# devmentality/LEAStereo

Hardware: AMD Instinct MI355X
Metric: stereo pairs/s at 576×960 D=192, 1/2/4/8 GPU; EPE vs reference (higher is better)
Workload: dtype f32; 1 GPU; SceneFlow 576x960 D=192 fp32, batch 1 per GPU (BASELINE configs[1]); height=576, width=960, maxdisp=192, global_batch=1, parallelism=dp1 (pairs sharded over ranks, no collective in the step), launch=hip graph replay

## Files before the change

### include/leastereo_hip.h

```cpp
#ifndef LEASTEREO_HIP_H
#define LEASTEREO_HIP_H

#include <stddef.h>
#include <stdint.h>

#ifdef __cplusplus
extern "C" {
#endif

#define LEA_ABI_VERSION 14

#define LEA_F32 0
#define LEA_BF16 1

#define LEA_OK 0
#define LEA_E_INVALID 1001
#define LEA_E_UNSUPPORTED 1002

#define LEA_RELU 1u
#define LEA_RESIDUAL 2u
#define LEA_PAIR_SUM 4u

int lea_abi_version(void);
const char* lea_last_error(void);
// ... 15 lines not shown
                      unsigned flags, int dtype, void* stream);

int lea_conv3d_bnrelu_resampled(const void* x, int64_t x_bstride, int Di, int Hi, int Wi,
                                const float* w_packed, const float* scale, const float* shift,
                                const void* residual, int64_t r_bstride,
                                void* y, int64_t y_bstride,
                                int B, int cin, int cout, int D, int H, int W, int k,
                                unsigned flags, int dtype, void* stream);

int lea_conv3d_bnrelu_costvolume(const void* left, const void* right, int64_t f_bstride,
                                 const float* w_packed, const float* scale, const float* shift,
                                 void* y, int64_t y_bstride, int B, int C, int cout, int D3,
                                 int H, int W, unsigned flags, int dtype, void* stream);
const char* lea_conv3d_costvolume_kernel_name(int B, int cout, int D3, int H, int W);

const char* lea_conv3d_kernel_name(int B, int cout, int D, int H, int W, int k, int resampled);


size_t lea_conv2d_packed_floats(int cout, int cin);
int lea_conv2d_pack_weights(const float* w, float* packed, int cout, int cin, void* stream);

int lea_conv2d_bnrelu(const void* x, int64_t x_bstride, const float* w_packed,
                      const float* scale, const float* shift, const void* residual,
                      int64_t r_bstride, void* y, int64_t y_bstride, int B, int cin, int cout,
                      int H, int W, unsigned flags, int dtype, void* stream);

const char* lea_conv2d_kernel_name(int B, int cout, int H, int W);

int lea_conv2d_bnrelu_pair(const void* x, int64_t x_bstride, const float* w_packed,
                           const float* scale, const float* shift, const void* residual,
                           int64_t r_bstride, void* y, int64_t y_bstride, void* y2,
                           int64_t y2_bstride, int B, int cin, int cout, int c1, int H, int W,
                           unsigned flags, void* stream);

int lea_conv2d_s3_bnrelu(const void* x, int64_t x_bstride, const float* w, const float* scale,
                         const float* shift, void* y, int64_t y_bstride, int B, int cin, int cout,
                         int Hi, int Wi, unsigned flags, int dtype, void* stream);

int lea_feature_stem_bnrelu(const float* x, int64_t x_bstride, const float* w0, const float* scale0,
                            const float* shift0, const float* w1, const float* scale1,
                            const float* shift1, void* y, int64_t y_bstride, int B, int cin, int c0,
                            int c1, int Hi, int Wi, int dtype, void* stream);


int lea_resample3d_trilinear(const void* x, int64_t x_bstride, void* y, int64_t y_bstride,
                             int B, int C, int Di, int Hi, int Wi, int Do, int Ho, int Wo,
                             int align_corners, const float* scale, const float* shift,
                             unsigned flags, int dtype, void* stream);

size_t lea_tapsum_workspace_bytes(int B, int cout, int Hi, int Wi, int Do);
int lea_tapsum_upsample(const void* q, int64_t q_bstride, void* y, int64_t y_bstride,
                        int B, int cout, int Di, int Hi, int Wi, int Do, int Ho, int Wo,
                        const float* scale, const float* shift, unsigned flags,
                        void* workspace, int dtype, void* stream);

int lea_disparity_regression(const void* cost, float* disp, int B, int D3, int H3, int W3,
                             int maxdisp, int dtype, void* stream);

int lea_disparity_regression_stats(const void* cost, float* disp, float* entropy, float* peak,
                                   float* disp_local, int B, int D3, int H3, int W3, int maxdisp,
                                   int radius, int dtype, void* stream);

int lea_disparity_regression_right(const void* cost, float* disp_right, int B, int D3, int H3,
                                   int W3, int maxdisp, int dtype, void* stream);

int lea_disparity_lr_check(const float* disp_left, const float* disp_right, uint8_t* state,
// ... 220 lines not shown
```

### include/leastereo_hip_tuning.h

```cpp
#ifndef LEASTEREO_HIP_TUNING_H
#define LEASTEREO_HIP_TUNING_H

#ifdef __cplusplus
extern "C" {
#endif

int lea_conv3d_set_tile_override(int nt, int tw, int td);

int lea_conv3d_set_rs_gather(int on);

int lea_conv1x1_set_vector(int on);

int lea_conv3d_bf16_set_tile_override(int th, int td, int mt);

int lea_conv3d_bf16_set_variant(int variant);

int lea_conv3d_bf16_set_stream1x1(int on);

int lea_conv3d_bf16_set_pair_split(int on);

int lea_resample_bf16_set_batch(int k);

int lea_resample_bf16_set_cols(int on);

int lea_resample_set_mode(int mode);

int lea_conv2d_set_small(int on);

const char* lea_conv2d_kernel_name_cin(int B, int cin, int cout, int H, int W);

int lea_disparity_set_register_form(int on);

int lea_tapsum_set_rows(int on);

int lea_staged_rows(int Hi, int Ho, int ac, int R, int halo);

int lea_conv3d_wino_set_w22(int on);

int lea_conv3d_wino_set_tile_override(int np, int td, int f);

int lea_conv3d_wino_set_variant(int variant);

int lea_conv3d_wino2_set_walk(int spw);

int lea_conv3d_wino2_set_halo16(int on);

int lea_conv3d_wino2_set_lane_halo16(int on);

int lea_conv3d_wino_set_fence(int on);

int lea_conv3d_wino2_set_pipeline(int on);

int lea_conv3d_wino2p_set_wpre(int on);

int lea_conv3d_wino44_set(int on);

int lea_conv3d_wino44_set_upre(int on);

int lea_conv3d_wino44_set_sched(int s);

int lea_conv3d_wino44_set_group(int g);

// ... 11 lines not shown
```

### leastereo_amd/_lib.py

```python
from __future__ import annotations

import ctypes
import os
import threading

LIB_PATH = os.environ.get(
    "LEASTEREO_HIP_LIB",
    os.path.join(os.path.dirname(os.path.abspath(__file__)), "libleastereo_hip.so"))

ABI_VERSION = 14
LEA_F32 = 0
LEA_BF16 = 1
LEA_RELU = 1
LEA_RESIDUAL = 2
LEA_PAIR_SUM = 4
LEA_E_INVALID = 1001

_p = ctypes.c_void_p
_i = ctypes.c_int
_i64 = ctypes.c_int64
_u = ctypes.c_uint

SIGNATURES = {
    "lea_abi_version": (_i, []),
# ... 75 lines not shown
    "lea_from_c8_bf16": (_i, [_p, _i64, _p, _i64, _i, _i, _i64, _p]),
    "lea_conv3d_wino_packed_floats": (ctypes.c_size_t, [_i, _i]),
    "lea_conv3d_wino_pack_weights": (_i, [_p, _p, _i, _i, _p]),
    "lea_conv3d_bnrelu_wino": (_i, [_p, _i64, _p, _i64, _i, _p, _p, _p, _p, _i64, _p, _i64,
                                    _i, _i, _i, _i, _i, _i, _u, _i, _p]),
    "lea_conv3d_bnrelu_costvolume_wino": (_i, [_p, _p, _i64, _p, _p, _p, _p, _i64, _i, _i, _i,
                                               _i, _i, _i, _u, _i, _p]),
    "lea_conv3d_wino_kernel_name": (ctypes.c_char_p, [_i, _i, _i, _i, _i, _i, _i]),
    "lea_conv3d_wino_down2_supported": (_i, [_i, _i, _i, _i, _i, _i]),
    "lea_conv3d_wino_down2_kernel_name": (ctypes.c_char_p, [_i, _i, _i, _i, _i, _i]),
    "lea_conv3d_bnrelu_wino_down2": (_i, [_p, _i64, _p, _p, _p, _p, _i64, _i, _i, _i, _i, _i, _i, _u, _i, _p]),
    "lea_conv3d_wino_down2_cat_supported": (_i, [_i, _i, _i, _i, _i, _i, _i]),
    "lea_conv3d_wino_down2_cat_kernel_name": (ctypes.c_char_p, [_i, _i, _i, _i, _i, _i, _i]),
    "lea_conv3d_bnrelu_wino_down2_cat": (_i, [_p, _i64, _p, _i64, _i, _p, _p, _p, _p, _i64, _i, _i, _i, _i, _i, _i,
                                              _u, _i, _p]),
    "lea_conv3d_wino_dp_down2_supported": (_i, [_i, _i, _i, _i, _i, _i]),
    "lea_conv3d_wino_dp_down2_kernel_name": (ctypes.c_char_p, [_i, _i, _i, _i, _i, _i, _i]),
    "lea_conv3d_bnrelu_wino_dp_down2": (_i, [_p, _i64, _p, _p, _p, _p, _i64, _p, _i64, _p, _i64, _i, _i, _i, _i, _i,
                                             _i, _u, _i, _p]),
    "lea_resample3d_down2_supported": (_i, [_i, _i, _i, _i, _i, _i, _i]),
    "lea_resample3d_trilinear_down2": (_i, [_p, _i64, _p, _i64, _p, _i64, _i, _i, _i, _i, _i, _i, _i, _i, _p, _p,
                                            _u, _i, _p]),
    "lea_conv3d_wino_set_tile_override": (_i, [_i, _i, _i]),
    "lea_conv3d_wino_set_variant": (_i, [_i]),
    "lea_conv3d_wino2_set_walk": (_i, [_i]),
    "lea_conv3d_wino2_set_halo16": (_i, [_i]),
    "lea_conv3d_wino2_set_lane_halo16": (_i, [_i]),
    "lea_conv3d_wino_set_fence": (_i, [_i]),
    "lea_resample_set_mode": (_i, [_i]),
    "lea_conv2d_set_small": (_i, [_i]),
    "lea_conv2d_kernel_name_cin": (ctypes.c_char_p, [_i, _i, _i, _i, _i]),
    "lea_conv2d_bnrelu_pair": (_i, [_p, _i64, _p, _p, _p, _p, _i64, _p, _i64, _p, _i64, _i, _i, _i, _i, _i,
                                    _i, _u, _p]),
    "lea_conv3d_wino2_set_pipeline": (_i, [_i]),
    "lea_conv3d_wino2p_set_wpre": (_i, [_i]),
    "lea_conv3d_wino44_set": (_i, [_i]),
    "lea_conv3d_wino44_set_upre": (_i, [_i]),
    "lea_conv3d_wino44_set_sched": (_i, [_i]),
    "lea_conv3d_wino44_set_group": (_i, [_i]),
    "lea_conv3d_wino_set_epi_buf": (_i, [_i]),
    "lea_conv3d_set_rs_gather": (_i, [_i]),
    "lea_conv1x1_set_vector": (_i, [_i]),
    "lea_conv3d_bf16_set_stream1x1": (_i, [_i]),
    "lea_conv3d_wino_set_small_cout": (_i, [_i]),
    "lea_conv3d_wino_set_block48": (_i, [_i]),
    "lea_cv_stem_split_weights": (_i, [_p, _p, _p, _i, _i, _p]),
    "lea_cv_stem_combine": (_i, [_p, _i64, _p, _i64, _p, _p, _p, _i64, _i, _i, _i, _i, _i, _u, _i,
                                 _p]),
    "lea_cv_stem_down2_supported": (_i, [_i, _i, _i, _i, _i]),
    "lea_cv_stem_combine_down2": (_i, [_p, _i64, _p, _i64, _p, _p, _p, _i64, _p, _i64, _i, _i, _i, _i, _i,
                                       _u, _i, _p]),
    "lea_standardize_workspace_bytes": (ctypes.c_size_t, [_i]),
    "lea_standardize_crop_u8": (_i, [_p, _p, _i, _i, _i, _i, _p, _p, _i, _i, _p, _p]),
    "lea_train_transform_workspace_bytes": (ctypes.c_size_t, [_i]),
    "lea_train_transform_u8": (_i, [_p, _p, _i, _i, _i, _i, _p, _p, _p, _p, _p, _p, _i, _i,
                                    ctypes.c_float, _p, _p, _p]),
    "lea_standardize_tiles_workspace_bytes": (ctypes.c_size_t, []),
    "lea_standardize_tiles_u8": (_i, [_p, _p, _i, _i, _i, _p, _i, _p, _p, _i, _i, _p, _p]),
    "lea_tile_blend_f32": (_i, [_p, _i64, _p, _i, _p, _i, _i, _i, _i, _i, _i, _i, _i, _p, _i, _i, _p, _p]),
    "lea_disparity_metrics_workspace_bytes": (ctypes.c_size_t, [_i, _i, _i]),
    "lea_disparity_metrics": (_i, [_p, _i64, _p, _i64, _i, _i, _i, ctypes.c_float, _i, _i,
                                   _i, _i, _i, _p, _p, _p, _p]),
    "lea_conv3d_wgrad_workspace_bytes": (ctypes.c_size_t, [_i, _i, _i, _i, _i, _i, _i]),
    "lea_conv3d_wgrad": (_i, [_p, _p, _p, _p, ctypes.c_size_t, _i, _i, _i, _i, _i, _i, _i, _p]),
    "lea_conv2d_wgrad_workspace_bytes": (ctypes.c_size_t, [_i, _i, _i, _i, _i]),
    "lea_conv2d_wgrad": (_i, [_p, _p, _p, _p, ctypes.c_size_t, _i, _i, _i, _i, _i, _p]),
# ... 77 lines not shown
```

### leastereo_amd/csrc/conv2d_small.hip

```cpp
#include <algorithm>

#include "common.h"
#include "conv3d_impl.h"

namespace lea {

constexpr int kSmallTW = 32;
constexpr int kSmallRS = kSmallTW + 2;

template <int CIN, int NG>
__global__ __launch_bounds__(256) void conv2d_small_kernel(const ConvArgs a) {
  constexpr int TH = 8 / NG;
  constexpr int MT = NG == 4 ? 2 : 1;
  using P = PackCfg<3, MT, 1>;
  constexpr int PL = (TH + 2) * kSmallRS;
  constexpr int CO8 = NG * 8;
  __shared__ float xs[CIN * PL];
  __shared__ __attribute__((aligned(16))) float ws[CIN * 9 * CO8];
  __shared__ float ss[2 * CO8];
  const int tid = threadIdx.x;
  const int tx = tid & 31;
  const int rest = tid >> 5;
  const int ty = rest % TH;
  const int cg = __builtin_amdgcn_readfirstlane(rest / TH);
  const int b = blockIdx.z;
  const int w0 = blockIdx.x * kSmallTW, h0 = blockIdx.y * TH;
  const long long HW = (long long)a.H * a.W;
  const float* xb = a.x + (long long)b * a.xbs;
  float xv[(CIN * PL + 255) / 256];
#pragma unroll
  for (int k = 0; k < (CIN * PL + 255) / 256; ++k) {
    const int e = tid + 256 * k;
    const int ci = e / PL, r = e - ci * PL;
    const int rr = r / kSmallRS, cc = r - rr * kSmallRS;
    const int h = h0 - 1 + rr, w = w0 - 1 + cc;
    const bool ok = e < CIN * PL && ci < a.cin && (unsigned)h < (unsigned)a.H && (unsigned)w < (unsigned)a.W;
    const int cic = min(ci, a.cin - 1), hc = min(max(h, 0), a.H - 1), wc = min(max(w, 0), a.W - 1);
    const float v = xb[cic * HW + (long long)hc * a.W + wc];
    xv[k] = ok ? v : 0.f;
  }
  float wv[(CIN * 9 * CO8 + 255) / 256];
#pragma unroll
  for (int k = 0; k < (CIN * 9 * CO8 + 255) / 256; ++k) {
    const int e = min(tid + 256 * k, CIN * 9 * CO8 - 1);
    const int co = e % CO8, q = e / CO8, tap = q % 9, ci = q / 9;
    const int ch = ci / P::CIN_B, cb = ci % P::CIN_B;
    const int col = (P::SWZ && (cb & 1)) ? (co ^ 16) : co;
    wv[k] = a.wp[((ch * 9 + tap) * P::CIN_B + cb) * P::COP + col];
  }
  if (tid < 2 * CO8) {
    const int coc = min(tid % CO8, a.cout - 1);
    ss[tid] = a.scale ? (tid < CO8 ? a.scale[coc] : a.shift[coc]) : (tid < CO8 ? 1.f : 0.f);
  }
#pragma unroll
  for (int k = 0; k < (CIN * PL + 255) / 256; ++k)
    if (tid + 256 * k < CIN * PL) xs[tid + 256 * k] = xv[k];
#pragma unroll
  for (int k = 0; k < (CIN * 9 * CO8 + 255) / 256; ++k)
    if (tid + 256 * k < CIN * 9 * CO8) ws[tid + 256 * k] = wv[k];
  __syncthreads();
  float acc[8];
#pragma unroll
  for (int j = 0; j < 8; ++j) acc[j] = 0.f;
  const float* xp = xs + ty * kSmallRS + tx;
  const float4* wq = reinterpret_cast<const float4*>(ws) + cg * 2;
#pragma unroll 1
  for (int ci = 0; ci < CIN; ++ci) {
#pragma unroll
    for (int tap = 0; tap < 9; ++tap) {
      const float v = xp[ci * PL + (tap / 3) * kSmallRS + tap % 3];
      const float4 wa = wq[(ci * 9 + tap) * (CO8 / 4)], wb = wq[(ci * 9 + tap) * (CO8 / 4) + 1];
      const float wr[8] = {wa.x, wa.y, wa.z, wa.w, wb.x, wb.y, wb.z, wb.w};
#pragma unroll
      for (int j = 0; j < 8; ++j) acc[j] = fmaf(wr[j], v, acc[j]);
    }
  }
  const int h = h0 + ty, w = w0 + tx;
  const bool second = a.csplit > 0 && cg * 8 >= a.csplit;
  const bool relu = a.flags & LEA_RELU, resid = (a.flags & LEA_RESIDUAL) && !second;
  const long long pix = (long long)min(h, a.H - 1) * a.W + min(w, a.W - 1);
  float rv[8], sc[8], sh[8];
#pragma unroll
  for (int j = 0; j < 8; ++j) {
    const int coc = min(cg * 8 + j, a.cout - 1);
    sc[j] = ss[cg * 8 + j];
    sh[j] = ss[CO8 + cg * 8 + j];
    rv[j] = resid ? a.res[(long long)b * a.rbs + coc * HW + pix] : 0.f;
  }
#pragma unroll
  for (int j = 0; j < 8; ++j) {
    float v = acc[j];
    v = v * sc[j] + sh[j];
    if (relu) v = fmaxf(v, 0.f);
    acc[j] = resid ? v + rv[j] : v;
  }
  if (h >= a.H || w >= a.W) return;
  float* yp = second ? a.y2 + (long long)b * a.y2bs + pix - (long long)a.csplit * HW : a.y + (long long)b * a.ybs + pix;
  if (cg * 8 + 8 <= a.cout) {
#pragma unroll
    for (int j = 0; j < 8; ++j) yp[(cg * 8 + j) * HW] = acc[j];
  } else {
#pragma unroll
    for (int j = 0; j < 8; ++j)
      if (cg * 8 + j < a.cout) yp[(cg * 8 + j) * HW] = acc[j];
  }
}

int g_conv2d_small = 1;

bool conv2d_small_ok(int cin, int cout) { return g_conv2d_small && cin <= 16 && cout <= 32; }

static int ng_of(int cout) { return cout <= 8 ? 1 : cout <= 16 ? 2 : 4; }

const char* conv2d_small_name(int cin, int cout) {
  static thread_local char name[64];
  snprintf(name, sizeof(name), "conv2d_small_kernel<%d, %d>", (cin + 3) / 4 * 4, ng_of(cout));
  return name;
}

int run_conv2d_small(const ConvArgs& a, int B, hipStream_t st) {
  const int ng = ng_of(a.cout), cin4 = (a.cin + 3) / 4 * 4, th = 8 / ng;
  LEA_CHECK_ARG(B <= 65535 && (a.H + th - 1) / th <= 65535, "lea_conv2d: grid too large");
  const dim3 grid((a.W + kSmallTW - 1) / kSmallTW, (a.H + th - 1) / th, B);
#define LEA_SMALL2D(CI, G)                                                      \
  if (cin4 == CI && ng == G) {                                                  \
    conv2d_small_kernel<CI, G><<<grid, 256, 0, st>>>(a);                        \
    return launch_status("lea_conv2d(small)");                                  \
  }
// ... 70 lines not shown
```

### leastereo_amd/executor.py

```python
from __future__ import annotations

import os
from dataclasses import dataclass

import torch

from . import kernels
from .arch import scale_dimension


def _stacked(fl: torch.Tensor, fr: torch.Tensor) -> torch.Tensor:
    if (fl.is_contiguous() and fr.is_contiguous() and fl.shape == fr.shape and fl.dtype == fr.dtype
            and fl.device == fr.device
            and fl.untyped_storage().data_ptr() == fr.untyped_storage().data_ptr()
            and fr.data_ptr() == fl.data_ptr() + fl.numel() * fl.element_size()):
        return fl.as_strided((2 * fl.shape[0],) + tuple(fl.shape[1:]), fl.stride())
    return torch.cat((fl, fr), 0)


@dataclass
class ConvParams:
    packed: torch.Tensor
    scale: torch.Tensor | None
    shift: torch.Tensor | None
    cin: int
    cout: int
    k: int
    relu: bool
    kind: str = "3d"
    wino: torch.Tensor | None = None


WINOGRAD = os.environ.get("LEASTEREO_WINOGRAD", "1") != "0"
CV_STEM = os.environ.get("LEASTEREO_CV_STEM", "1") != "0"


def _conv_params(mod, w=None, folded=None):
    w = mod.conv.weight if w is None else w
    scale, shift = mod.folded_bn() if folded is None else folded
    cout, cin, k = w.shape[0], w.shape[1], w.shape[-1]
    if w.dim() == 5:
        return ConvParams(kernels.pack_conv_weight(w), scale, shift, cin, cout, k, mod.relu)
    if k == 1:
        return ConvParams(kernels.pack_conv_weight(w.reshape(cout, cin, 1, 1, 1)), scale, shift,
                          cin, cout, 1, mod.relu)
    if mod.stride == 3:
        return ConvParams(w.detach().contiguous(), scale, shift, cin, cout, 3, mod.relu, "s3")
    if mod.stride != 1 or mod.padding != 1:
        raise ValueError(f"unsupported Conv2d stride={mod.stride} padding={mod.padding}")
    return ConvParams(kernels.pack_conv2d_weight(w), scale, shift, cin, cout, 3, mod.relu, "2d")


class CellGraphExecutor:

    tap = None

    def _emit(self, name, t):
        if self.tap is not None:
            self.tap(name, self._as_f32(t))

    @staticmethod
    def _as_f32(t):
        return t.detach().clone()

    SHARE_DOWNSAMPLE = os.environ.get("LEASTEREO_SHARE_DOWNSAMPLE", "1") != "0"
    SPLIT_S1_GROUP48 = False
    PAIR_S0 = False
    PAIR_STEPS = False
    PAIR_C = tuple(int(c) for c in os.environ.get("LEASTEREO_PAIR_C", "8,16,32").split(",") if c)

    def __init__(self, net):
        from .model import ConvBR
        self.m = net
        self.p = {}
        with torch.no_grad():
            for name, mod in net.named_modules():
                if isinstance(mod, ConvBR):
                    self.p[name] = _conv_params(mod)
            self.s1_group = {}
            self.s1_split = set()
            for i, cell in enumerate(net.cells):
                group = []
                for k, terms in enumerate(cell.plan):
                    for op, j in terms:
                        if j == 1 and cell.op_kinds[op] == "conv":
                            group.append((k, op))
                            break
                first_cat_state = 2 + cell.steps - cell.block_multiplier
                steps = [k for k, _ in group]
                if (len(group) < 2 or steps != list(range(steps[0], steps[0] + len(steps)))
                        or 2 + steps[0] < first_cat_state):
                    continue
                mods = [cell._ops[op] for _, op in group]
                split = (self.SPLIT_S1_GROUP48 and WINOGRAD and len(mods) == 3 and cell.c_out == 16
                         and mods[0].conv.weight.dim() == 5 and mods[0].conv.weight.shape[2] == 3)
                for key, part in ((("s1_group_head", mods[:1]), ("s1_group", mods[1:])) if split
                                  else (("s1_group", mods),)):
                    w = torch.cat([m.conv.weight for m in part], 0)
                    folded = [m.folded_bn() for m in part]
                    scale = torch.cat([f[0] for f in folded]).contiguous()
                    shift = torch.cat([f[1] for f in folded]).contiguous()
                    self.p[f"cells.{i}.{key}"] = _conv_params(part[0], w, (scale, shift))
                self.s1_group[i] = group
                if split:
                    self.s1_split.add(i)
            self.s0_pair = {}
            for i, cell in enumerate(net.cells) if self.PAIR_S0 else ():
                pair = [(k, op) for k, terms in enumerate(cell.plan) for op, j in terms
                        if j == 0 and cell.op_kinds[op] == "conv"]
                first_cat_state = 2 + cell.steps - cell.block_multiplier
                if (len(pair) != 2 or getattr(cell, "dims", 3) != 2 or 2 + pair[0][0] < first_cat_state
                        or cell.c_out % 8 or 2 * cell.c_out > 32):
                    continue
                (k0, op0), (k1, op1) = pair
                m0, m1 = cell._ops[op0], cell._ops[op1]
                other = [(o, j) for o, j in cell.plan[k1] if o != op1]
                if {k for k, _ in self.s1_group.get(i, [])} & {k0, k1}:
                    continue
                if (m0.relu != m1.relu or m0.conv.weight.dim() != 4 or m0.conv.weight.shape[-1] != 3
                        or m0.stride != 1 or m1.stride != 1 or cell.plan[k1][0][0] != op1
                        or not other or cell.op_kinds[other[0][0]] != "conv"):
                    continue
                w = torch.cat([m0.conv.weight, m1.conv.weight], 0)
                folded = [m0.folded_bn(), m1.folded_bn()]
                self.p[f"cells.{i}.s0_pair"] = _conv_params(
                    m0, w, (torch.cat([f[0] for f in folded]).contiguous(),
                            torch.cat([f[1] for f in folded]).contiguous()))
                self.s0_pair[i] = pair
            self.pair_steps = {}
            for i, cell in enumerate(net.cells) if self.PAIR_STEPS else ():
                terms = [[(op, j) for op, j in t] for t in cell.plan]
                if (getattr(cell, "dims", 3) != 3 or not terms or cell.c_out not in self.PAIR_C
                        or any(len(t) != 2 or any(cell.op_kinds[op] != "conv" for op, _ in t) for t in terms)):
                    continue
                mods = [[cell._ops[op] for op, _ in t] for t in terms]
                if any(m.conv.weight.shape[-1] != 3 or not m.relu for ms in mods for m in ms):
                    continue
                for k, (ma, mb) in enumerate(mods):
                    folded = [ma.folded_bn(), mb.folded_bn()]
                    self.p[f"cells.{i}.pair{k}"] = self._pair_params(
                        ma, torch.cat([ma.conv.weight, mb.conv.weight], 1),
                        (torch.cat([f[0] for f in folded]).contiguous(),
                         torch.cat([f[1] for f in folded]).contiguous()))
                self.pair_steps[i] = terms
            cells = list(net.cells)
            for i, (cell, nxt) in enumerate(zip(cells, cells[1:])):
                if (self.SHARE_DOWNSAMPLE and cell.downup_sample != 0 and nxt.downup_sample == 0
                        and nxt.c_out == cell.c_out and 2 + cell.steps - cell.block_multiplier == 1
                        and cell.preprocess.conv.weight.shape[1] == nxt.pre_preprocess.conv.weight.shape[1]
                        and cell.preprocess.conv.weight.shape[1] != nxt.c_out):
                    mods = [nxt.pre_preprocess, cell.preprocess]
                    folded = [m.folded_bn() for m in mods]
                    self.p[f"cells.{i}.share"] = _conv_params(
                        mods[0], torch.cat([m.conv.weight for m in mods], 0),
                        (torch.cat([f[0] for f in folded]).contiguous(),
                         torch.cat([f[1] for f in folded]).contiguous()))

    def conv(self, name, x, out=None, accumulate=False, x2=None, size=None, residual=None, down=None,
             down_only=False):
        p = self.p[name]
        cin = x.shape[1] + (x2.shape[1] if x2 is not None else 0)
# ... 58 lines not shown
                    cell = self.m.cells[i]
                    w = torch.cat([cell._ops[op].conv.weight for op, _ in self.pair_steps[i][k]], 1)
                elif name.endswith("s1_group") or name.endswith("s1_group_head"):
                    i = int(name.split(".")[1])
                    mods = [self.m.cells[i]._ops[op] for _, op in self.s1_group[i]]
                    if i in self.s1_split:
                        mods = mods[:1] if name.endswith("_head") else mods[1:]
                    w = torch.cat([m.conv.weight for m in mods], 0)
                else:
                    w = self.m.get_submodule(name).conv.weight
                p.wino = kernels.pack_conv_weight_wino(w)

    def _empty(self, b, c, size, like):
        return torch.empty((b, c) + tuple(size), device=like.device, dtype=like.dtype)

    @staticmethod
    def _channels(t, c0, c1):
        return t[:, c0:c1]

    @staticmethod
    def _nchannels(t):
        return t.shape[1]

    @staticmethod
    def _volume(t):
        return tuple(t.shape[2:5])

    @staticmethod
    def _resample(x, size):
        return kernels.resample_trilinear(x, size)

    def _cell_output_takes_down(self, i, size):
        return False

    def cell(self, i, s0, s1, down=None):
        cell = self.m.cells[i]
        c = cell.c_out
        if down is not None and down[0] is not None:
            s0 = down[0]
        s1_down = down is not None and down[1] is not None
        if s1_down:
            s1 = down[1]
        prev_input = s1
        size = self._volume(s1)
        if cell.downup_sample != 0 and not s1_down:
            sc = 0.5 if cell.downup_sample < 0 else 2
            size = tuple(n if (cell.dims == 2 and ax == 0) else scale_dimension(n, sc)
                         for ax, n in enumerate(size))
        b = s1.shape[0]
        bm = cell.block_multiplier
        n_states = 2 + cell.steps
        memo, self._share_memo = getattr(self, "_share_memo", None), None
        share = f"cells.{i}.share" in self.p
        if share:
            big = self._empty(b, c + bm * c, size, s1)
            out = self._channels(big, c, c + bm * c)
        else:
            out = self._empty(b, bm * c, size, s1)
        slot = {idx: self._channels(out, k * c, (k + 1) * c)
                for k, idx in enumerate(range(n_states - bm, n_states))}
        dn = None
        if self._cell_output_takes_down(i, size) and self._down_kernels_take(s1, c, self._volume(s1), size):
            dn = self._empty(b, bm * c, tuple(n // 2 for n in size), s1)
        self._cell_down = dn
        dslot = {} if dn is None else {idx: self._channels(dn, k * c, (k + 1) * c) for k, idx in enumerate(slot)}
        group = self.s1_group.get(i, [])
        if memo is not None and memo[0] is s0 and memo[1] == size:
            s0 = memo[2]
            if 0 in slot:
                slot[0].copy_(s0)
        elif self._nchannels(s0) != c:
            s0 = self.conv(f"cells.{i}.pre_preprocess", s0, out=slot.get(0), size=size)
        else:
            if self._volume(s0) != size:
                s0 = self._resample(s0, size)
            if 0 in slot:
                slot[0].copy_(s0)
        if share:
            self.conv(f"cells.{i}.share", s1, out=self._channels(big, 0, 2 * c), size=size)
            self._share_memo = (prev_input, size, self._channels(big, 0, c))
            s1 = self._channels(big, c, 2 * c)
        else:
            s1 = self.conv(f"cells.{i}.preprocess", s1, out=slot.get(1), size=size,
                           **({} if dn is None else {"down": dslot[1]}))
        states = [s0, s1]
        pairs = self.pair_steps.get(i)
        if pairs is not None:
            dsts = [slot.get(2 + k) for k in range(len(pairs))]
            if all(d is not None for d in dsts) and all(
                    self._pair_ok(states[t[0][1]] if t[0][1] < 2 else dsts[t[0][1] - 2],
                                  states[t[1][1]] if t[1][1] < 2 else dsts[t[1][1] - 2], dsts[k])
                    for k, t in enumerate(pairs)):
                for k, ((_, ja), (_, jb)) in enumerate(pairs):
                    self.pair_conv(f"cells.{i}.pair{k}", states[ja], states[jb], dsts[k])
                    states.append(dsts[k])
                return prev_input, out
        written = set()
        done = set(group)
        consumed = set()
        pair = self.s0_pair.get(i)
        if pair is not None and self._nchannels(s0) == c and self._volume(s0) == size:
            (k0, op0), (k1, op1) = pair
            skips0 = [states[j] for o, j in cell.plan[k0] if cell.op_kinds[o] != "conv"]
            p = self.p[f"cells.{i}.s0_pair"]
            kernels.conv2d_bnrelu_pair(s0, p.packed, c, 2 * c, p.scale, p.shift, p.relu,
                                       slot[2 + k0], slot[2 + k1], skips0[-1] if skips0 else None)
            done |= {(k0, op0), (k1, op1)}
            written |= {k0, k1}
            if skips0:
                consumed.add(k0)
        if group:
            k0 = 2 + group[0][0] - (n_states - bm)
            if i in self.s1_split:
                self.conv(f"cells.{i}.s1_group", s1, out=self._channels(out, (k0 + 1) * c, (k0 + 3) * c))
                self.conv(f"cells.{i}.s1_group_head", s1, out=self._channels(out, k0 * c, (k0 + 1) * c))
            else:
                self.conv(f"cells.{i}.s1_group", s1, out=self._channels(out, k0 * c, (k0 + len(group)) * c))
            written |= {k for k, _ in group}
        for step, terms in enumerate(cell.plan):
            dst = slot.get(len(states))
            if dst is None:
                dst = self._empty(b, c, size, s1)
            skips = [states[j] for k, j in terms if cell.op_kinds[k] != "conv"]
            if step in consumed:
                skips.pop()
            todo = [k for k, _ in terms if (step, k) not in done and cell.op_kinds[k] == "conv"]
            for k, j in terms:
                if (step, k) in done or cell.op_kinds[k] != "conv":
                    continue
# ... 169 lines not shown
    def _last3_same_size(self, last):
        return self.conv("last_3", last)

    def __init__(self, matching):
        super().__init__(matching)
        with torch.no_grad():
            last3 = matching.last_3.conv.weight
            co, ci = last3.shape[:2]
            taps = last3.permute(0, 2, 3, 4, 1).reshape(co * 27, ci, 1, 1, 1)
            self.p["last_3.taps"] = ConvParams(kernels.pack_conv_weight(taps), None, None,
                                               ci, co * 27, 1, False)
            self.cv = None
            if CV_STEM:
                self.cv = self._cv_stem_pack(*kernels.cv_stem_split_weights(matching.stem0.conv.weight))
        self._use_winograd()


class MatchingExecutorDirect(MatchingExecutor):

    SPLIT_S1_GROUP48 = False
    PAIR_STEPS = False

    def __init__(self, matching):
        super().__init__(matching)
        self.cv = None

    def _use_winograd(self):
        """Direct engine only."""


class FeatureExecutor(CellGraphExecutor):
    FUSED_STEM = os.environ.get("LEASTEREO_FEATURE_STEM", "1") != "0"
    PAIR_S0 = os.environ.get("LEASTEREO_PAIR_S0", "1") != "0"

    def _stems(self, x, c8=False, x2=None):
        p0, p1 = self.p["stem0"], self.p["stem1"]
        if (self.FUSED_STEM and p0.relu and p1.relu and (p0.cin, p0.cout, p1.cout) == (3, 16, 32)
                and p1.kind == "s3"):
            return kernels.feature_stem(x, self.m.stem0.conv.weight, p0.scale, p0.shift, p1.packed,
                                        p1.scale, p1.shift, c8, x2)
        if x2 is not None:
            x = torch.cat((x, x2), 0)
        stem1 = self.conv("stem1", self.conv("stem0", x.unsqueeze(2)))
        return kernels.to_c8(stem1) if c8 else stem1

    def run(self, x, x2=None):
        stem1 = self._stems(x, x2=x2)
        stem2 = self.conv("stem2", stem1)
        out = (stem1, stem2)
        for i in range(len(self.m.cells)):
            out = self.cell(i, out[0], out[1])
        last = out[-1]
        h, w = stem2.shape[3:]
        lh = last.shape[3]
        full, half, quarter = (1, h, w), (1, h // 2, w // 2), (1, h // 4, w // 4)
        if lh == h:
            y = last
        elif lh == h // 2:
            y = kernels.resample_trilinear(self.conv("last_6", last), full)
        elif lh == h // 4:
            y = self.conv("last_6", self.conv("last_12", last), size=half)
            y = kernels.resample_trilinear(y, full)
        elif lh == h // 8:
            y = self.conv("last_12", self.conv("last_24", last), size=quarter)
            y = kernels.resample_trilinear(self.conv("last_6", y, size=half), full)
        else:
# ... 232 lines not shown
```

### leastereo_amd/kernels.py

```python
from __future__ import annotations

import collections
import contextlib
import math
import os

import numpy as np
import torch

from . import _lib
from ._lib import LEA_F32, LEA_PAIR_SUM, LEA_RELU, LEA_RESIDUAL, check


def _stream():
    return torch.cuda.current_stream().cuda_stream


class KernelProbe:

    def __init__(self, names=None):
        self.names = None if names is None else set(names)
        self.records = []

    def __enter__(self):
# ... 266 lines not shown
        "lea_conv2d_bnrelu")
    _probe_end(rec)
    return out


def conv2d_bnrelu_pair(x: torch.Tensor, packed: torch.Tensor, c1: int, cout: int,
                       scale: torch.Tensor | None, shift: torch.Tensor | None, relu: bool,
                       out1: torch.Tensor, out2: torch.Tensor,
                       residual: torch.Tensor | None = None) -> None:
    _require_cuda(x, packed, scale, shift, out1, out2, residual)
    b, cin, d, h, w = x.shape
    if d != 1:
        raise ValueError("conv2d_bnrelu_pair takes [B, C, 1, H, W] views")
    xbs = _check_volume_view(x, "x")
    if tuple(out1.shape) != (b, c1, 1, h, w) or tuple(out2.shape) != (b, cout - c1, 1, h, w):
        raise ValueError(f"conv2d_bnrelu_pair: outputs {tuple(out1.shape)} / {tuple(out2.shape)}")
    y1bs, y2bs = _check_volume_view(out1, "out1"), _check_volume_view(out2, "out2")
    rptr, rbs = None, 0
    if residual is not None:
        if tuple(residual.shape) != tuple(out1.shape):
            raise ValueError(f"conv2d_bnrelu_pair: residual {tuple(residual.shape)}")
        rbs = _check_volume_view(residual, "residual")
        rptr = residual.data_ptr()
    flags = (LEA_RELU if relu else 0) | (LEA_RESIDUAL if rptr is not None else 0)
    rec = None if _probe is None else _probe_launch(
        conv2d_kernel_name(b, cout, h, w, cin), 2.0 * b * h * w * cout * cin * 9,
        4.0 * b * h * w * (cin + cout + (c1 if rptr is not None else 0)) + 36.0 * cout * cin)
    check(_lib.load().lea_conv2d_bnrelu_pair(
        x.data_ptr(), xbs, packed.data_ptr(),
        scale.data_ptr() if scale is not None else None,
        shift.data_ptr() if shift is not None else None,
        rptr, rbs, out1.data_ptr(), y1bs, out2.data_ptr(), y2bs, b, cin, cout, c1, h, w, flags, _stream()),
        "lea_conv2d_bnrelu_pair")
    _probe_end(rec)


def feature_stem(x: torch.Tensor, w0: torch.Tensor, scale0, shift0, w1: torch.Tensor, scale1, shift1,
                 c8: bool = False, x2: torch.Tensor | None = None) -> torch.Tensor:
    _require_cuda(x, x2, scale0, shift0, scale1, shift1)
    w0, w1 = w0.detach().contiguous(), w1.detach().contiguous()
    _require_cuda(w0, w1)
    x = x.contiguous()
    srcs = [x]
    if x2 is not None:
        if tuple(x2.shape) != tuple(x.shape):
            raise ValueError(f"feature_stem: x2 {tuple(x2.shape)} differs from x {tuple(x.shape)}")
        x2 = x2.contiguous()
        srcs.append(x2)
    b, cin, hi, wi = x.shape
    c0, c1 = w0.shape[0], w1.shape[0]
    if tuple(w0.shape) != (c0, cin, 3, 3) or tuple(w1.shape) != (c1, c0, 3, 3):
        raise ValueError(f"feature_stem: weights {tuple(w0.shape)} / {tuple(w1.shape)} do not chain")
    ho, wo = (hi - 1) // 3 + 1, (wi - 1) // 3 + 1
    nb = b * len(srcs)
    if c8:
        out = torch.empty((nb, c1 // 8, 1, ho, wo, 8), device=x.device, dtype=torch.bfloat16)
    else:
        out = torch.empty((nb, c1, 1, ho, wo), device=x.device, dtype=torch.float32)
    ptr = lambda t: t.data_ptr() if t is not None else None
    if len(srcs) == 2 and b == 1:
        srcs, b, xbs = [x], 2, (x2.data_ptr() - x.data_ptr()) // x.element_size()
    else:
        xbs = x.stride(0)
    rec = None if _probe is None else _probe_launch(
        "feature_stem_kernel", 2.0 * nb * ho * wo * (9 * 9 * cin * c0 + 9 * c0 * c1),
        4.0 * nb * cin * hi * wi + out.numel() * out.element_size(), 0.0)
# ... 1362 lines not shown
```

Before: 163.8 pairs/s.

## Fuse a whole 2D feature cell's five convs into one tiled kernel

```diff
diff --git a/include/leastereo_hip.h b/include/leastereo_hip.h
--- a/include/leastereo_hip.h
+++ b/include/leastereo_hip.h
@@ -71,6 +71,12 @@
                            int64_t r_bstride, void* y, int64_t y_bstride, void* y2,
                            int64_t y2_bstride, int B, int cin, int cout, int c1, int H, int W,
                            unsigned flags, void* stream);
+
+int lea_conv2d_cell_fused_supported(int B, int c, int H, int W);
+int lea_conv2d_cell_fused(const void* s0, int64_t s0_bstride, const void* s1, int64_t s1_bstride,
+                          const float* w_packed, const float* scale, const float* shift, void* y2,
+                          int64_t y2_bstride, void* y3, int64_t y3_bstride, void* y4,
+                          int64_t y4_bstride, int B, int c, int H, int W, void* stream);
 
 int lea_conv2d_s3_bnrelu(const void* x, int64_t x_bstride, const float* w, const float* scale,
                          const float* shift, void* y, int64_t y_bstride, int B, int cin, int cout,
diff --git a/include/leastereo_hip_tuning.h b/include/leastereo_hip_tuning.h
--- a/include/leastereo_hip_tuning.h
+++ b/include/leastereo_hip_tuning.h
@@ -28,6 +28,8 @@
 int lea_conv2d_set_small(int on);
 
 const char* lea_conv2d_kernel_name_cin(int B, int cin, int cout, int H, int W);
+
+int lea_conv2d_cell_set_tile(int c, int tile);
 
 int lea_disparity_set_register_form(int on);
 
diff --git a/leastereo_amd/_lib.py b/leastereo_amd/_lib.py
--- a/leastereo_amd/_lib.py
+++ b/leastereo_amd/_lib.py
@@ -131,6 +131,10 @@
     "lea_conv2d_kernel_name_cin": (ctypes.c_char_p, [_i, _i, _i, _i, _i]),
     "lea_conv2d_bnrelu_pair": (_i, [_p, _i64, _p, _p, _p, _p, _i64, _p, _i64, _p, _i64, _i, _i, _i, _i, _i,
                                     _i, _u, _p]),
+    "lea_conv2d_cell_fused_supported": (_i, [_i, _i, _i, _i]),
+    "lea_conv2d_cell_fused": (_i, [_p, _i64, _p, _i64, _p, _p, _p, _p, _i64, _p, _i64, _p, _i64, _i, _i, _i, _i,
+                                   _p]),
+    "lea_conv2d_cell_set_tile": (_i, [_i, _i]),
     "lea_conv3d_wino2_set_pipeline": (_i, [_i]),
     "lea_conv3d_wino2p_set_wpre": (_i, [_i]),
     "lea_conv3d_wino44_set": (_i, [_i]),
diff --git a/leastereo_amd/csrc/conv2d_cell.hip b/leastereo_amd/csrc/conv2d_cell.hip
--- /dev/null
+++ b/leastereo_amd/csrc/conv2d_cell.hip
@@ -0,0 +1,253 @@
+#include <algorithm>
+
+#include "common.h"
+#include "conv2d_small.h"
+#include "conv3d_impl.h"
+
+namespace lea {
+
+struct CellArgs {
+  const float* s0;
+  long long s0bs;
+  const float* s1;
+  long long s1bs;
+  const float* wp;
+  const float* scale;
+  const float* shift;
+  float* y[3];
+  long long ybs[3];
+  int H, W;
+};
+
+template <int C, int RW, int RH, int NT>
+__device__ __forceinline__ void cell_window_load(float (&v)[(C * RW * RH + NT - 1) / NT], const float* src,
+                                                 long long HW, int H, int W, int hb, int wb, int tid) {
+  constexpr int PL = RW * RH;
+#pragma unroll
+  for (int k = 0; k < (C * PL + NT - 1) / NT; ++k) {
+    const int e = tid + NT * k;
+    const int ci = e / PL, r = e - ci * PL;
+    const int rr = r / RW, cc = r - rr * RW;
+    const int h = hb + rr, w = wb + cc;
+    const bool ok = e < C * PL && (unsigned)h < (unsigned)H && (unsigned)w < (unsigned)W;
+    const int cic = min(ci, C - 1), hc = min(max(h, 0), H - 1), wc = min(max(w, 0), W - 1);
+    const float x = src[cic * HW + (long long)hc * W + wc];
+    v[k] = ok ? x : 0.f;
+  }
+}
+
+template <int N, int NT>
+__device__ __forceinline__ void cell_window_store(float* dst, const float (&v)[(N + NT - 1) / NT], int tid) {
+#pragma unroll
+  for (int k = 0; k < (N + NT - 1) / NT; ++k)
+    if (tid + NT * k < N) dst[tid + NT * k] = v[k];
+}
+
+template <int C, int TW, int TH, int NT, int P>
+__global__ __launch_bounds__(NT) void conv2d_cell_kernel(const CellArgs a) {
+  constexpr int NG = C / 8;
+  constexpr int W0 = TW + 6, H0 = TH + 6;
+  constexpr int W1 = TW + 4, H1 = TH + 4;
+  constexpr int W3 = TW + 2, H3 = TH + 2;
+  constexpr int PL0 = W0 * H0, PL1 = W1 * H1, PL3 = W3 * H3;
+  constexpr int NW = C * 9 * C;
+  constexpr int PAD = (P - 1) * W0;
+  __shared__ float x0[C * PL0 + PAD], x1[C * PL1 + PAD], x2[C * PL1 + PAD], x3[C * PL3 + PAD];
+  __shared__ __attribute__((aligned(16))) float ws[5 * NW];
+  __shared__ float ss[10 * C];
+  const int tid = threadIdx.x;
+  const int b = blockIdx.z;
+  const int w0 = blockIdx.x * TW, h0 = blockIdx.y * TH;
+  const int H = a.H, W = a.W;
+  const long long HW = (long long)H * W;
+  {
+    using PK = PackCfg<3, 1, 1>;
+    constexpr int KW = (5 * NW + NT - 1) / NT;
+    float v0[(C * PL0 + NT - 1) / NT], v1[(C * PL1 + NT - 1) / NT], wv[KW];
+    cell_window_load<C, W0, H0, NT>(v0, a.s0 + (long long)b * a.s0bs, HW, H, W, h0 - 3, w0 - 3, tid);
+    cell_window_load<C, W1, H1, NT>(v1, a.s1 + (long long)b * a.s1bs, HW, H, W, h0 - 2, w0 - 2, tid);
+#pragma unroll
+    for (int k = 0; k < KW; ++k) {
+      const int e = min(tid + NT * k, 5 * NW - 1);
+      const int op = e / NW, q = e - op * NW;
+      const int co = q % C, tap = (q / C) % 9, ci = q / (9 * C);
+      wv[k] = a.wp[op * (C / 4) * PK::CHUNK + ((ci / 4 * 9 + tap) * PK::CIN_B + ci % 4) * PK::COP + co];
+    }
+    for (int e = tid; e < 10 * C; e += NT) ss[e] = e < 5 * C ? a.scale[e] : a.shift[e - 5 * C];
+    cell_window_store<C * PL0, NT>(x0, v0, tid);
+    cell_window_store<C * PL1, NT>(x1, v1, tid);
+    cell_window_store<5 * NW, NT>(ws, wv, tid);
+  }
+  __syncthreads();
+  const float4* wq = reinterpret_cast<const float4*>(ws);
+  float* const y2 = a.y[0] + (long long)b * a.ybs[0];
+  float* const y3 = a.y[1] + (long long)b * a.ybs[1];
+  float* const y4 = a.y[2] + (long long)b * a.ybs[2];
+
+  {
+    constexpr int NS = (H1 + P - 1) / P;
+#pragma unroll 1
+    for (int it = tid; it < NG * NS * W1; it += NT) {
+      const int g = it / (NS * W1), r = it - g * (NS * W1);
+      const int sy = r / W1, rx = r - sy * W1, ry = sy * P;
+      float acc[P][8] = {};
+      small_dot8<C, P, PL0, W0, C / 4>(x0 + ry * W0 + rx, wq + 0 * NW / 4 + g * 2, acc);
+      const int w = w0 - 2 + rx;
+#pragma unroll
+      for (int p = 0; p < P; ++p) {
+        const int row = ry + p, h = h0 - 2 + row;
+        if (row >= H1) continue;
+        const bool in = (unsigned)h < (unsigned)H && (unsigned)w < (unsigned)W;
+        const bool mine = in && row >= 2 && row < TH + 2 && rx >= 2 && rx < TW + 2;
+#pragma unroll
+        for (int j = 0; j < 8; ++j) {
+          const int co = g * 8 + j;
+          float v = small_epilogue(acc[p][j], ss[co], ss[5 * C + co], true, true, x1[co * PL1 + row * W1 + rx]);
+          v = in ? v : 0.f;
+          x2[co * PL1 + row * W1 + rx] = v;
+          if (mine) y2[co * HW + (long long)h * W + w] = v;
+        }
+      }
+    }
+  }
+  __syncthreads();
+  {
+    constexpr int NS = (H3 + P - 1) / P;
+#pragma unroll 1
+    for (int it = tid; it < NG * NS * W3; it += NT) {
+      const int g = it / (NS * W3), r = it - g * (NS * W3);
+      const int sy = r / W3, rx = r - sy * W3, ry = sy * P;
+      float t[P][8] = {}, acc[P][8] = {};
+      small_dot8<C, P, PL1, W1, C / 4>(x1 + ry * W1 + rx, wq + 1 * NW / 4 + g * 2, t);
+      small_dot8<C, P, PL1, W1, C / 4>(x2 + ry * W1 + rx, wq + 2 * NW / 4 + g * 2, acc);
+      const int w = w0 - 1 + rx;
+#pragma unroll
+      for (int p = 0; p < P; ++p) {
+        const int row = ry + p, h = h0 - 1 + row;
+        if (row >= H3) continue;
+        const bool in = (unsigned)h < (unsigned)H && (unsigned)w < (unsigned)W;
+        const bool mine = in && row >= 1 && row < TH + 1 && rx >= 1 && rx < TW + 1;
+#pragma unroll
+        for (int j = 0; j < 8; ++j) {
+          const int co = g * 8 + j;
+          const float u = small_epilogue(t[p][j], ss[C + co], ss[6 * C + co], true, false, 0.f);
+          float v = small_epilogue(acc[p][j], ss[2 * C + co], ss[7 * C + co], true, true, u);
+          v = in ? v : 0.f;
+          x3[co * PL3 + row * W3 + rx] = v;
+          if (mine) y3[co * HW + (long long)h * W + w] = v;
+        }
+      }
+    }
+  }
+  __syncthreads();
+  {
+    constexpr int NS = (TH + P - 1) / P;
+#pragma unroll 1
+    for (int it = tid; it < NG * NS * TW; it += NT) {
+      const int g = it / (NS * TW), r = it - g * (NS * TW);
+      const int sy = r / TW, rx = r - sy * TW, ry = sy * P;
+      float t[P][8] = {}, acc[P][8] = {};
+      small_dot8<C, P, PL0, W0, C / 4>(x0 + (ry + 2) * W0 + rx + 2, wq + 3 * NW / 4 + g * 2, t);
+      small_dot8<C, P, PL3, W3, C / 4>(x3 + ry * W3 + rx, wq + 4 * NW / 4 + g * 2, acc);
+      const int w = w0 + rx;
+#pragma unroll
+      for (int p = 0; p < P; ++p) {
+        const int h = h0 + ry + p;
+        if (ry + p >= TH || h >= H || w >= W) continue;
+#pragma unroll
+        for (int j = 0; j < 8; ++j) {
+          const int co = g * 8 + j;
+          const float u = small_epilogue(t[p][j], ss[3 * C + co], ss[8 * C + co], true, false, 0.f);
+          y4[co * HW + (long long)h * W + w] =
+              small_epilogue(acc[p][j], ss[4 * C + co], ss[9 * C + co], true, true, u);
+        }
+      }
+    }
+  }
+}
+
+static int g_cell_tile[2] = {1, 1};
+
+struct CellTile {
+  int tw, th;
+};
+
+static bool cell_tile_of(int c, CellTile* t) {
+  const int v = c == 8 ? g_cell_tile[0] : c == 16 ? g_cell_tile[1] : 0;
+  if (v == 0) return false;
+  if (c == 8) *t = v == 1 ? CellTile{32, 8} : CellTile{32, 16};
+  else *t = v == 1 ? CellTile{16, 8} : CellTile{16, 16};
+  return true;
+}
+
+constexpr int kCellCUs = 256;
+
+static bool cell_fused_ok(int B, int c, int H, int W) {
+  CellTile t;
+  if (!(conv2d_small_ok(c, c) && B > 0 && H > 0 && W > 0 && cell_tile_of(c, &t))) return false;
+  const long long tiles = (long long)((W + t.tw - 1) / t.tw) * ((H + t.th - 1) / t.th) * B;
+  return B <= 65535 && (H + t.th - 1) / t.th <= 65535 && (long long)(4 * c + 63) * H * W < (1LL << 31) &&
+         (c == 8 || tiles <= kCellCUs);
+}
+
+}
+
+extern "C" int lea_conv2d_cell_set_tile(int c, int tile) {
+  lea::clear_error();
+  if ((c != 8 && c != 16) || tile < 0 || tile > 2) {
+    lea::set_error("lea_conv2d_cell_set_tile: c=%d tile=%d", c, tile);
+    return LEA_E_INVALID;
+  }
+  lea::g_cell_tile[c == 16] = tile;
+  return 0;
+}
+
+extern "C" int lea_conv2d_cell_fused_supported(int B, int c, int H, int W) {
+  return lea::cell_fused_ok(B, c, H, W) ? 1 : 0;
+}
+
+extern "C" int lea_conv2d_cell_fused(const void* s0, int64_t s0_bstride, const void* s1, int64_t s1_bstride,
+                                     const float* w_packed, const float* scale, const float* shift, void* y2,
+                                     int64_t y2_bstride, void* y3, int64_t y3_bstride, void* y4,
+                                     int64_t y4_bstride, int B, int c, int H, int W, void* stream) {
+  using namespace lea;
+  clear_error();
+  LEA_CHECK_ARG(s0 && s1 && w_packed && scale && shift && y2 && y3 && y4, "lea_conv2d_cell_fused: null pointer");
+  LEA_CHECK_ARG(B > 0 && c > 0 && H > 0 && W > 0, "lea_conv2d_cell_fused: bad shape B=%d c=%d H=%d W=%d", B, c, H, W);
+  const void* io[5] = {s0, s1, y2, y3, y4};
+  for (int i = 0; i < 5; ++i)
+    for (int j = std::max(i + 1, 2); j < 5; ++j)
+      LEA_CHECK_ARG(io[i] != io[j], "lea_conv2d_cell_fused: an output aliases another tensor");
+  if (!cell_fused_ok(B, c, H, W)) {
+    set_error("lea_conv2d_cell_fused: B=%d c=%d H=%d W=%d not taken (c = 8, or 16 within one round of tiles, on "
+              "the few-channel tile)", B, c, H, W);
+    return LEA_E_UNSUPPORTED;
+  }
+  CellArgs a{};
+  a.s0 = (const float*)s0;
+  a.s0bs = s0_bstride;
+  a.s1 = (const float*)s1;
+  a.s1bs = s1_bstride;
+  a.wp = w_packed;
+  a.scale = scale;
+  a.shift = shift;
+  a.y[0] = (float*)y2, a.y[1] = (float*)y3, a.y[2] = (float*)y4;
+  a.ybs[0] = y2_bstride, a.ybs[1] = y3_bstride, a.ybs[2] = y4_bstride;
+  a.H = H;
+  a.W = W;
+  CellTile t;
+  cell_tile_of(c, &t);
+  const dim3 grid((W + t.tw - 1) / t.tw, (H + t.th - 1) / t.th, B);
+  const int v = g_cell_tile[c == 16];
+  hipStream_t st = as_stream(stream);
+#define LEA_CELL2D(CC, V, TW, TH, NT, P)                           \
+  if (c == CC && v == V) {                                         \
+    conv2d_cell_kernel<CC, TW, TH, NT, P><<<grid, NT, 0, st>>>(a); \
+    return launch_status("lea_conv2d_cell_fused");                 \
+  }
+  LEA_CELL2D(8, 1, 32, 8, 256, 2) LEA_CELL2D(8, 2, 32, 16, 512, 2)
+  LEA_CELL2D(16, 1, 16, 8, 256, 2) LEA_CELL2D(16, 2, 16, 16, 512, 2)
+#undef LEA_CELL2D
+  set_error("lea_conv2d_cell_fused: c=%d tile=%d", c, v);
+  return LEA_E_UNSUPPORTED;
+}
diff --git a/leastereo_amd/csrc/conv2d_small.h b/leastereo_amd/csrc/conv2d_small.h
--- /dev/null
+++ b/leastereo_amd/csrc/conv2d_small.h
@@ -0,0 +1,30 @@
+#pragma once
+
+namespace lea {
+
+template <int CIN, int P, int PL, int RS, int W4>
+__device__ __forceinline__ void small_dot8(const float* xp, const float4* wq, float (&acc)[P][8]) {
+#pragma unroll 1
+  for (int ci = 0; ci < CIN; ++ci) {
+#pragma unroll
+    for (int tap = 0; tap < 9; ++tap) {
+      float v[P];
+#pragma unroll
+      for (int p = 0; p < P; ++p) v[p] = xp[ci * PL + (tap / 3 + p) * RS + tap % 3];
+      const float4 wa = wq[(ci * 9 + tap) * W4], wb = wq[(ci * 9 + tap) * W4 + 1];
+      const float wr[8] = {wa.x, wa.y, wa.z, wa.w, wb.x, wb.y, wb.z, wb.w};
+#pragma unroll
+      for (int p = 0; p < P; ++p)
+#pragma unroll
+        for (int j = 0; j < 8; ++j) acc[p][j] = fmaf(wr[j], v[p], acc[p][j]);
+    }
+  }
+}
+
+__device__ __forceinline__ float small_epilogue(float v, float sc, float sh, bool relu, bool resid, float rv) {
+  v = v * sc + sh;
+  if (relu) v = fmaxf(v, 0.f);
+  return resid ? v + rv : v;
+}
+
+}
diff --git a/leastereo_amd/csrc/conv2d_small.hip b/leastereo_amd/csrc/conv2d_small.hip
--- a/leastereo_amd/csrc/conv2d_small.hip
+++ b/leastereo_amd/csrc/conv2d_small.hip
@@ -1,6 +1,7 @@
 #include <algorithm>
 
 #include "common.h"
+#include "conv2d_small.h"
 #include "conv3d_impl.h"
 
 namespace lea {
@@ -59,22 +60,12 @@
   for (int k = 0; k < (CIN * 9 * CO8 + 255) / 256; ++k)
     if (tid + 256 * k < CIN * 9 * CO8) ws[tid + 256 * k] = wv[k];
   __syncthreads();
-  float acc[8];
+  float accp[1][8];
+  float(&acc)[8] = accp[0];
 #pragma unroll
   for (int j = 0; j < 8; ++j) acc[j] = 0.f;
-  const float* xp = xs + ty * kSmallRS + tx;
-  const float4* wq = reinterpret_cast<const float4*>(ws) + cg * 2;
-#pragma unroll 1
-  for (int ci = 0; ci < CIN; ++ci) {
-#pragma unroll
-    for (int tap = 0; tap < 9; ++tap) {
-      const float v = xp[ci * PL + (tap / 3) * kSmallRS + tap % 3];
-      const float4 wa = wq[(ci * 9 + tap) * (CO8 / 4)], wb = wq[(ci * 9 + tap) * (CO8 / 4) + 1];
-      const float wr[8] = {wa.x, wa.y, wa.z, wa.w, wb.x, wb.y, wb.z, wb.w};
-#pragma unroll
-      for (int j = 0; j < 8; ++j) acc[j] = fmaf(wr[j], v, acc[j]);
-    }
-  }
+  small_dot8<CIN, 1, PL, kSmallRS, CO8 / 4>(xs + ty * kSmallRS + tx, reinterpret_cast<const float4*>(ws) + cg * 2,
+                                            accp);
   const int h = h0 + ty, w = w0 + tx;
   const bool second = a.csplit > 0 && cg * 8 >= a.csplit;
   const bool relu = a.flags & LEA_RELU, resid = (a.flags & LEA_RESIDUAL) && !second;
@@ -88,12 +79,7 @@
     rv[j] = resid ? a.res[(long long)b * a.rbs + coc * HW + pix] : 0.f;
   }
 #pragma unroll
-  for (int j = 0; j < 8; ++j) {
-    float v = acc[j];
-    v = v * sc[j] + sh[j];
-    if (relu) v = fmaxf(v, 0.f);
-    acc[j] = resid ? v + rv[j] : v;
-  }
+  for (int j = 0; j < 8; ++j) acc[j] = small_epilogue(acc[j], sc[j], sh[j], relu, resid, rv[j]);
   if (h >= a.H || w >= a.W) return;
   float* yp = second ? a.y2 + (long long)b * a.y2bs + pix - (long long)a.csplit * HW : a.y + (long long)b * a.ybs + pix;
   if (cg * 8 + 8 <= a.cout) {
diff --git a/leastereo_amd/executor.py b/leastereo_amd/executor.py
--- a/leastereo_amd/executor.py
+++ b/leastereo_amd/executor.py
@@ -51,6 +51,19 @@
     return ConvParams(kernels.pack_conv2d_weight(w), scale, shift, cin, cout, 3, mod.relu, "2d")
 
 
+_FUSED_CELL_PLAN = [[(0, 0), (1, 1)], [(2, 1), (3, 2)], [(4, 0), (5, 3)]]
+_FUSED_CELL_KINDS = ["conv", "skip", "conv", "conv", "conv", "conv"]
+_FUSED_CELL_OPS = (0, 2, 3, 4, 5)
+
+
+def fused_cell2d_ops(cell):
+    plan = [[(int(op), int(j)) for op, j in terms] for terms in cell.plan]
+    if (getattr(cell, "dims", 3) != 2 or cell.steps != 3 or cell.block_multiplier != 4
+            or plan != _FUSED_CELL_PLAN or list(cell.op_kinds) != _FUSED_CELL_KINDS):
+        return None
+    return _FUSED_CELL_OPS
+
+
 class CellGraphExecutor:
 
     tap = None
@@ -66,6 +79,7 @@
     SHARE_DOWNSAMPLE = os.environ.get("LEASTEREO_SHARE_DOWNSAMPLE", "1") != "0"
     SPLIT_S1_GROUP48 = False
     PAIR_S0 = False
+    FUSED_CELL = False
     PAIR_STEPS = False
     PAIR_C = tuple(int(c) for c in os.environ.get("LEASTEREO_PAIR_C", "8,16,32").split(",") if c)
 
@@ -127,6 +141,16 @@
                     m0, w, (torch.cat([f[0] for f in folded]).contiguous(),
                             torch.cat([f[1] for f in folded]).contiguous()))
                 self.s0_pair[i] = pair
+            self.fused_cell = {}
+            for i in self.s0_pair:
+                ops = fused_cell2d_ops(net.cells[i])
+                ps = [self.p[f"cells.{i}._ops.{k}"] for k in ops or ()]
+                c = net.cells[i].c_out
+                if ops is None or not all(p.kind == "2d" and p.relu and p.scale is not None
+                                          and (p.cin, p.cout, p.k) == (c, c, 3) for p in ps):
+                    continue
+                self.fused_cell[i] = (torch.cat([p.packed.reshape(-1) for p in ps]),
+                                      torch.cat([p.scale for p in ps]), torch.cat([p.shift for p in ps]))
             self.pair_steps = {}
             for i, cell in enumerate(net.cells) if self.PAIR_STEPS else ():
                 terms = [[(op, j) for op, j in t] for t in cell.plan]
@@ -251,6 +275,11 @@
 
     def _cell_output_takes_down(self, i, size):
         return False
+
+    def _cell_takes_fused2d(self, i, s0, c, size):
+        return (self.FUSED_CELL and self.PAIR_S0 and self.tap is None and not isinstance(self, _C8Layout)
+                and i in self.s0_pair and i in self.fused_cell and self._nchannels(s0) == c
+                and self._volume(s0) == size and kernels.conv2d_cell_fused_supported(s0, c))
 
     def cell(self, i, s0, s1, down=None):
         cell = self.m.cells[i]
@@ -314,6 +343,9 @@
                     self.pair_conv(f"cells.{i}.pair{k}", states[ja], states[jb], dsts[k])
                     states.append(dsts[k])
                 return prev_input, out
+        if self._cell_takes_fused2d(i, s0, c, size) and dn is None and all(k in slot for k in (2, 3, 4)):
+            kernels.conv2d_cell_fused(s0, s1, *self.fused_cell[i], slot[2], slot[3], slot[4])
+            return prev_input, out
         written = set()
         done = set(group)
         consumed = set()
@@ -549,6 +581,7 @@
 class FeatureExecutor(CellGraphExecutor):
     FUSED_STEM = os.environ.get("LEASTEREO_FEATURE_STEM", "1") != "0"
     PAIR_S0 = os.environ.get("LEASTEREO_PAIR_S0", "1") != "0"
+    FUSED_CELL = os.environ.get("LEASTEREO_FUSED_CELL2D", "1") != "0"
 
     def _stems(self, x, c8=False, x2=None):
         p0, p1 = self.p["stem0"], self.p["stem1"]
diff --git a/leastereo_amd/kernels.py b/leastereo_amd/kernels.py
--- a/leastereo_amd/kernels.py
+++ b/leastereo_amd/kernels.py
@@ -322,6 +322,37 @@
         shift.data_ptr() if shift is not None else None,
         rptr, rbs, out1.data_ptr(), y1bs, out2.data_ptr(), y2bs, b, cin, cout, c1, h, w, flags, _stream()),
         "lea_conv2d_bnrelu_pair")
+    _probe_end(rec)
+
+
+def conv2d_cell_fused_supported(s0: torch.Tensor, c: int) -> bool:
+    if not s0.is_cuda or s0.dtype != torch.float32 or s0.dim() != 5 or s0.shape[2] != 1:
+        return False
+    b, _, _, h, w = s0.shape
+    return bool(_lib.load().lea_conv2d_cell_fused_supported(b, c, h, w))
+
+
+def conv2d_cell_fused(s0: torch.Tensor, s1: torch.Tensor, packed: torch.Tensor, scale: torch.Tensor,
+                      shift: torch.Tensor, out2: torch.Tensor, out3: torch.Tensor, out4: torch.Tensor) -> None:
+    _require_cuda(s0, s1, packed, scale, shift, out2, out3, out4)
+    b, c, d, h, w = s0.shape
+    if d != 1:
+        raise ValueError("conv2d_cell_fused takes [B, C, 1, H, W] views")
+    for name, t in (("s1", s1), ("out2", out2), ("out3", out3), ("out4", out4)):
+        if tuple(t.shape) != tuple(s0.shape):
+            raise ValueError(f"conv2d_cell_fused: {name} {tuple(t.shape)} vs s0 {tuple(s0.shape)}")
+    if packed.numel() != 5 * _lib.load().lea_conv2d_packed_floats(c, c) or scale.numel() != 5 * c \
+            or shift.numel() != 5 * c or not (packed.is_contiguous() and scale.is_contiguous()
+                                               and shift.is_contiguous()):
+        raise ValueError("conv2d_cell_fused: parameters of five c -> c convs expected")
+    bs = [_check_volume_view(t, name) for name, t in (("s0", s0), ("s1", s1), ("out2", out2), ("out3", out3),
+                                                      ("out4", out4))]
+    rec = None if _probe is None else _probe_launch(
+        f"conv2d_cell_kernel<{c}>", 5 * 2.0 * b * h * w * c * c * 9, 4.0 * b * h * w * 5 * c + 5 * 36.0 * c * c)
+    check(_lib.load().lea_conv2d_cell_fused(
+        s0.data_ptr(), bs[0], s1.data_ptr(), bs[1], packed.data_ptr(), scale.data_ptr(), shift.data_ptr(),
+        out2.data_ptr(), bs[2], out3.data_ptr(), bs[3], out4.data_ptr(), bs[4], b, c, h, w, _stream()),
+        "lea_conv2d_cell_fused")
     _probe_end(rec)
 
 
```

Result: no change. 164.6 pairs/s, median of 6 (+0.4%).
